# fircarpediem/LSS2_Multimodal_nu

Hardware: AMD Instinct MI355X
Metric: BEV frames/sec (6-cam 352x128 -> 200x200x64), full hot path: CamEncode lift + splat + BevEncode (higher is better)
Workload: dtype bf16; 1 GPU; BASELINE configs[1]: model_BEV_TXT LSS hot path, batch=4/GPU, 6 cams 352x128, D=41, 200x200x64 BEV -> BevEncode -> 200x200x4, trunk (EfficientNet) not included: features are the input; batch_per_gpu=4, global_batch=4, parallelism=dp1 (sample-sharded, no collective), precision=bf16

## Files before the change

lss2_multimodal_nu_amd/csrc/conv_ring.hip:

```cpp
#include <stdlib.h>

#include <type_traits>

#include "lss_common.h"

namespace {

constexpr int RK_SW = 20, RK_SH = 4;
constexpr int RK_PW = 24, RK_PH = 6;
constexpr int RK_KC = 32;
constexpr int RK_POSB = RK_KC * 2;
constexpr int RK_STRIP_PATCH = RK_PH * RK_PW * RK_POSB;
constexpr int RK_SLAB = 128 * RK_KC * 2;
constexpr int RK_SRC_H = 5, RK_SRC_W = 14;
constexpr int RK_SRC_STRIP = RK_SRC_H * RK_SRC_W * RK_POSB;

struct RingArgs {
  const unsigned short* x;
  const unsigned short* x2;
  const unsigned char* w;
  const float* scale;
  const float* shift;
  unsigned short* y;
  const float* head_w;
  const float* head_b;
  float* head_out;
  int head_n;
  int B, H, W, Cx, C2, up, Hin, Win, Cin, Cout, relu, wt;
  float ry, rx;
  int SX, SY, nstrips, nblk, nch;
  unsigned long long* stats;
};

__device__ __attribute__((aligned(128))) unsigned char lss_ring_zero_page[128];
__device__ int lss_ring_timeouts;

template <int MODE, bool HEAD, int NSL>
struct RingLds {
  static constexpr int RING = 0;
  static constexpr int PATCH = NSL * RK_SLAB;
  static constexpr int SRC = PATCH + 2 * 4 * RK_STRIP_PATCH;
  static constexpr int HEADX = SRC + (MODE == 1 ? 4 * RK_SRC_STRIP : 0);
  static constexpr int FLAGS = HEADX + (HEAD ? 4 * 80 * 4 * 4 : 0);
  static constexpr int TOTAL = FLAGS + 256;
};
constexpr int F_FULL_W = 0, F_FREE_W = 8, F_FULL_P = 16, F_FREE_P = 18, F_HEAD = 20, F_FULL_S = 24, F_FREE_S = 25;

#define RK_TIMEOUT_COUNTER lss_ring_timeouts
#include "ring_prims.h"

typedef __attribute__((ext_vector_type(2))) float rk_f32x2;
typedef __attribute__((ext_vector_type(2))) __bf16 rk_bf16x2;
__device__ __forceinline__ unsigned int rk_pack_bf2(float lo, float hi) {
  const rk_f32x2 v = {lo, hi};
  return __builtin_bit_cast(unsigned int, __builtin_convertvector(v, rk_bf16x2));
}
__device__ __forceinline__ uint4 rk_blend(const uint4& q00, const uint4& q01, const uint4& q10, const uint4& q11,
                                          float lx, float ly) {
  const float w11 = lx * ly, w10 = ly - w11, w01 = lx - w11, w00 = 1.f - lx - ly + w11;
  const unsigned int* u00 = reinterpret_cast<const unsigned int*>(&q00);
  const unsigned int* u01 = reinterpret_cast<const unsigned int*>(&q01);
  const unsigned int* u10 = reinterpret_cast<const unsigned int*>(&q10);
  const unsigned int* u11 = reinterpret_cast<const unsigned int*>(&q11);
  uint4 out;
  unsigned int* o = reinterpret_cast<unsigned int*>(&out);
#pragma unroll
  for (int i = 0; i < 4; ++i) {
    float lo = __builtin_bit_cast(float, u00[i] << 16) * w00;
    float hi = __builtin_bit_cast(float, u00[i] & 0xffff0000u) * w00;
    lo = __builtin_fmaf(__builtin_bit_cast(float, u01[i] << 16), w01, lo);
    hi = __builtin_fmaf(__builtin_bit_cast(float, u01[i] & 0xffff0000u), w01, hi);
    lo = __builtin_fmaf(__builtin_bit_cast(float, u10[i] << 16), w10, lo);
    hi = __builtin_fmaf(__builtin_bit_cast(float, u10[i] & 0xffff0000u), w10, hi);
    lo = __builtin_fmaf(__builtin_bit_cast(float, u11[i] << 16), w11, lo);
    hi = __builtin_fmaf(__builtin_bit_cast(float, u11[i] & 0xffff0000u), w11, hi);
    o[i] = rk_pack_bf2(lo, hi);
  }
  return out;
}

#ifndef RK_PSLEEP
#define RK_PSLEEP 8
#endif
#ifndef RK_PRIO_C
#define RK_PRIO_C 0
#endif
#ifndef RK_PRIO_P
#define RK_PRIO_P 3
#endif
#ifndef RK_PRIO_W
#define RK_PRIO_W 2
#endif
constexpr int RK_NS = 4;
constexpr int RK_NCONS = 2 * RK_NS;
constexpr int RK_NPATCH = 3;
constexpr int RK_NWAVES = RK_NCONS + 1 + RK_NPATCH;
constexpr int RK_NPIECE = RK_NS * 9;

struct RingTile {
  int nb;
  int b[RK_NS], oy0[RK_NS], ox0[RK_NS];
  bool ok[RK_NS];
};

template <int MODE, bool HEAD, int NSL>
__global__ __launch_bounds__(RK_NWAVES * 64, 3) void conv_ring_kernel(RingArgs a) {
  using L = RingLds<MODE, HEAD, NSL>;
  constexpr int LA = NSL - 2;
  static_assert(NSL >= 3 && NSL <= 8, "ring depth");
  static_assert(L::TOTAL <= 160 * 1024, "LDS of one CU");
  __shared__ __attribute__((aligned(1024))) unsigned char smem[L::TOTAL];
  const int tid = threadIdx.x, lane = tid & 63;
  const int wave = __builtin_amdgcn_readfirstlane(tid >> 6);
  const rk_flag_t flags = (rk_flag_t)((__attribute__((address_space(3))) unsigned char*)smem + L::FLAGS);
  if (tid < 64) flags[tid] = 0;
  __syncthreads();
  int st0 = 0, st1 = 0;
#ifdef RK_STATS
#define RK_ST(x) x
  const unsigned long long t_entry = a.stats ? __builtin_amdgcn_s_memrealtime() : 0ull;
  auto write_stats = [&]() {
    if (a.stats != nullptr && lane == 0) {
      unsigned long long* o = a.stats + ((size_t)blockIdx.x * RK_NWAVES + wave) * 6;
      o[0] = (unsigned long long)st0; o[1] = (unsigned long long)st1;
      o[2] = __builtin_amdgcn_s_memrealtime() - t_entry; o[3] = t_entry;
    }
  };
#else
#define RK_ST(x)
  auto write_stats = [&]() {};
#endif

  RingTile T;
  {
    const int nwg = gridDim.x, bid = blockIdx.x;
    const int xcd = bid & 7, q8 = nwg >> 3, r8 = nwg & 7;
    const int t = (xcd < r8 ? xcd * (q8 + 1) : r8 * (q8 + 1) + (xcd - r8) * q8) + (bid >> 3);
    T.nb = t % a.nblk;
    const int quad = t / a.nblk;
#pragma unroll
    for (int s = 0; s < RK_NS; ++s) {
      int sid = RK_NS * quad + s;
      T.ok[s] = sid < a.nstrips;
      sid = min(sid, a.nstrips - 1);
      const int per = a.SX * a.SY;
      T.b[s] = sid / per;
      const int rem = sid - T.b[s] * per;
      const int sy = rem / a.SX;
      T.oy0[s] = sy * RK_SH;
      T.ox0[s] = (rem - sy * a.SX) * RK_SW;
    }
  }
  const int nsteps = a.nch * 9;

  if (wave == RK_NCONS) {
    __builtin_amdgcn_s_setprio(RK_PRIO_W);
    const unsigned char* wsrc = a.w + (size_t)T.nb * a.nch * 9 * RK_SLAB + lane * 16;
    int slot = 0, gen = 1, pslot = 0, pgen = 1, inflight = 0;
    auto publish_oldest = [&]() {
      switch (inflight) {
        case 1: rk_wait_vmcnt<0>(); break;
        case 2: rk_wait_vmcnt<8>(); break;
        case 3: rk_wait_vmcnt<16>(); break;
        case 4: rk_wait_vmcnt<24>(); break;
        case 5: rk_wait_vmcnt<32>(); break;
        case 6: rk_wait_vmcnt<40>(); break;
        default: rk_wait_vmcnt<48>(); break;
      }
      rk_set(flags + F_FULL_W + pslot, pgen, lane);
      if (++pslot == NSL) { pslot = 0; ++pgen; }
      --inflight;
    };
    for (int i = 0; i < nsteps; ++i) {
      if (gen > 1) {
        int spins = 0;
        while (rk_peek(flags + F_FREE_W + slot) < RK_NCONS * (gen - 1)) {
          if (inflight > 0) {
            publish_oldest();
          } else {
            __builtin_amdgcn_s_sleep(1);
            ++st0;
            if (++spins > RK_SPIN_LIMIT) {
              if (lane == 0) atomicAdd(&lss_ring_timeouts, 1);
              break;
            }
          }
        }
        asm volatile("" ::: "memory");
      }
      unsigned char* dst = smem + L::RING + slot * RK_SLAB;
#ifndef RK_DIAG_NOWDMA
#pragma unroll
      for (int k = 0; k < 8; ++k) rk_glds16(wsrc + (size_t)i * RK_SLAB + k * 1024, dst + k * 1024);
#endif
      ++inflight;
      if (inflight > LA) publish_oldest();
      if (++slot == NSL) { slot = 0; ++gen; }
    }
    while (inflight > 0) publish_oldest();
    rk_wait_vmcnt<0>();
    write_stats();
    return;
  }

  if (wave > RK_NCONS) {
    __builtin_amdgcn_s_setprio(RK_PRIO_P);
    const int pw = wave - RK_NCONS - 1;
    constexpr int NIT = RK_NPIECE / RK_NPATCH;
    const int nskip = MODE == 1 ? a.C2 / RK_KC : a.nch;
    const unsigned short* xfull = MODE == 1 ? a.x2 : a.x;
    const int cfull = MODE == 1 ? a.C2 : a.Cx;
    int poff[NIT];
    int g_off[MODE == 1 ? NIT : 1];
    unsigned int g_w[MODE == 1 ? NIT : 1];
    constexpr int NSRC = MODE == 1 ? (RK_NS * 5 + RK_NPATCH - 1) / RK_NPATCH : 1;
    int src_o[NSRC];
#pragma unroll
    for (int k = 0; k < NIT; ++k) {
      const int it = pw + k * RK_NPATCH;
      const int s = it / 9, pos = (it % 9) * 16 + (lane >> 2);
      const int prow = pos / RK_PW, pcol = pos - prow * RK_PW;
      const int piece = (lane & 3) ^ ((prow & 1) << 1);
      const int sb = s == 0 ? T.b[0] : s == 1 ? T.b[1] : s == 2 ? T.b[2] : T.b[3];
      const int soy = s == 0 ? T.oy0[0] : s == 1 ? T.oy0[1] : s == 2 ? T.oy0[2] : T.oy0[3];
      const int sox = s == 0 ? T.ox0[0] : s == 1 ? T.ox0[1] : s == 2 ? T.ox0[2] : T.ox0[3];
      const bool sok = s == 0 ? T.ok[0] : s == 1 ? T.ok[1] : s == 2 ? T.ok[2] : T.ok[3];
      const int iy = soy - 1 + prow, ix = sox - 1 + pcol;
      const bool in = sok && pcol < RK_SW + 2 && iy >= 0 && iy < a.Hin && ix >= 0 && ix < a.Win;
      poff[k] = (in && cfull > 0) ? ((sb * a.Hin + iy) * a.Win + ix) * cfull + piece * 8 : -1;
      if (MODE == 1) {
        g_off[k] = 0;
        g_w[k] = 0;
        if (in) {
          const int wy0 = (int)(a.ry * (float)max(soy - 1, 0)), wx0 = (int)(a.rx * (float)max(sox - 1, 0));
          const float sy = a.ry * (float)iy, sx = a.rx * (float)ix;
          const int y0 = (int)sy, x0 = (int)sx;
          const unsigned int wy = (unsigned int)((sy - (float)y0) * 65536.f + 0.5f);
          const unsigned int wx = (unsigned int)((sx - (float)x0) * 65536.f + 0.5f);
          g_w[k] = min(wx, 65535u) | (min(wy, 65535u) << 16);
          const int fl = (x0 < a.W - 1 ? 1 : 0) | (y0 < a.H - 1 ? 2 : 0) | 4;
          g_off[k] = ((((y0 - wy0) * RK_SRC_W + (x0 - wx0)) * 4 + piece) * 16) | fl;
        }
      }
    }
    if (MODE == 1) {
#pragma unroll
      for (int k = 0; k < NSRC; ++k) {
        const int it = pw + k * RK_NPATCH;
        const int s = min(it / 5, RK_NS - 1), q = (it % 5) * 64 + lane;
        const int pos = min(q >> 2, RK_SRC_H * RK_SRC_W - 1), part = q & 3;
        const int sr = pos / RK_SRC_W, sc = pos - sr * RK_SRC_W;
        const int sb = s == 0 ? T.b[0] : s == 1 ? T.b[1] : s == 2 ? T.b[2] : T.b[3];
        const int soy = s == 0 ? T.oy0[0] : s == 1 ? T.oy0[1] : s == 2 ? T.oy0[2] : T.oy0[3];
        const int sox = s == 0 ? T.ox0[0] : s == 1 ? T.ox0[1] : s == 2 ? T.ox0[2] : T.ox0[3];
        const int wy0 = (int)(a.ry * (float)max(soy - 1, 0)), wx0 = (int)(a.rx * (float)max(sox - 1, 0));
        src_o[k] = ((sb * a.H + min(wy0 + sr, a.H - 1)) * a.W + min(wx0 + sc, a.W - 1)) * a.Cx + part * 8;
      }
    }
    auto issue_full = [&](int c, int buf) {
      unsigned char* dst = smem + L::PATCH + buf * (RK_NS * RK_STRIP_PATCH);
#pragma unroll
      for (int k = 0; k < NIT; ++k) {
        const void* src = poff[k] >= 0 ? (const void*)(xfull + poff[k] + c * RK_KC) : (const void*)lss_ring_zero_page;
        rk_glds16(src, dst + (pw + k * RK_NPATCH) * 1024);
      }
    };
    if (MODE == 0) {
      issue_full(0, 0);
      if (a.nch > 1) {
        issue_full(1, 1);
        rk_wait_vmcnt<NIT>();
      } else {
        rk_wait_vmcnt<0>();
      }
      rk_add1(flags + F_FULL_P + 0, lane);
      for (int c = 0; c < a.nch; ++c) {
        if (c + 1 < a.nch) {
          rk_wait_vmcnt<0>();
          rk_add1(flags + F_FULL_P + ((c + 1) & 1), lane);
        }
        if (c + 2 < a.nch) {
          st0 += rk_wait_ge<RK_PSLEEP>(flags + F_FREE_P + (c & 1), RK_NCONS * ((c >> 1) + 1));
          issue_full(c + 2, c & 1);
        }
      }
    } else {
      auto issue_src = [&](int c) {
        const int cx = c * RK_KC - a.C2;
#pragma unroll
        for (int k = 0; k < NSRC; ++k) {
          const int it = pw + k * RK_NPATCH;
          if (it < RK_NS * 5 && (it % 5) * 64 + lane < RK_SRC_H * RK_SRC_W * 4)
            rk_glds16(a.x + src_o[k] + cx, smem + L::SRC + (it / 5) * RK_SRC_STRIP + (it % 5) * 1024);
        }
      };
      auto prepare = [&](int c) {
        if (c < nskip) {
          st0 += rk_wait_ge<RK_PSLEEP>(flags + F_FREE_P + (c & 1), RK_NCONS * (c >> 1));
          issue_full(c, c & 1);
        } else {
          st1 += rk_wait_ge(flags + F_FREE_S, RK_NPATCH * (c - nskip));
          issue_src(c);
        }
      };
      prepare(0);
      for (int c = 0; c < a.nch; ++c) {
        rk_wait_vmcnt<0>();
        if (c >= nskip) {
          rk_add1(flags + F_FULL_S, lane);
          st1 += rk_wait_ge(flags + F_FULL_S, RK_NPATCH * (c - nskip + 1));
          st0 += rk_wait_ge<RK_PSLEEP>(flags + F_FREE_P + (c & 1), RK_NCONS * (c >> 1));
          unsigned char* dst = smem + L::PATCH + (c & 1) * (RK_NS * RK_STRIP_PATCH);
          uint4 qa[4], qb[4];
          auto corners = [&](int k, uint4* q) {
            const int it = pw + k * RK_NPATCH;
            const unsigned char* p00 = smem + L::SRC + (it / 9) * RK_SRC_STRIP + (g_off[k] & 0xfff0);
            const int dx = (g_off[k] & 1) ? 4 * 16 : 0, dy = (g_off[k] & 2) ? RK_SRC_W * 4 * 16 : 0;
            q[0] = *reinterpret_cast<const uint4*>(p00);
#if defined(RK_DIAG_ONEREAD)
            q[1] = q[0]; q[2] = q[0]; q[3] = q[0];
            asm volatile("" : "+v"(q[1].x), "+v"(q[2].x), "+v"(q[3].x));
#else
            q[1] = *reinterpret_cast<const uint4*>(p00 + dx);
            q[2] = *reinterpret_cast<const uint4*>(p00 + dy);
            q[3] = *reinterpret_cast<const uint4*>(p00 + dy + dx);
#endif
          };
          auto finish = [&](int k, const uint4* q) {
            uint4 v = make_uint4(0, 0, 0, 0);
#ifndef RK_DIAG_NOBLEND
#if defined(RK_DIAG_READSONLY)
            v.x = q[0].x ^ q[1].x ^ q[2].x ^ q[3].x; v.y = q[0].y ^ q[1].y ^ q[2].y ^ q[3].y;
            v.z = q[0].z ^ q[1].z ^ q[2].z ^ q[3].z; v.w = q[0].w ^ q[1].w ^ q[2].w ^ q[3].w;
#else
            v = rk_blend(q[0], q[1], q[2], q[3], (float)(g_w[k] & 0xffff) * (1.f / 65536.f),
                         (float)(g_w[k] >> 16) * (1.f / 65536.f));
#endif
            const bool in = (g_off[k] & 4) != 0;
            v.x = in ? v.x : 0u; v.y = in ? v.y : 0u; v.z = in ? v.z : 0u; v.w = in ? v.w : 0u;
#endif
            *reinterpret_cast<uint4*>(dst + (pw + k * RK_NPATCH) * 1024 + lane * 16) = v;
          };
          corners(0, qa);
#pragma unroll
          for (int k = 0; k < NIT; k += 2) {
            corners(k + 1, qb);
            finish(k, qa);
            if (k + 2 < NIT) corners(k + 2, qa);
            finish(k + 1, qb);
          }
          rk_wait_lgkm0();
          rk_add1(flags + F_FREE_S, lane);
        }
        if (c + 1 < a.nch && c + 1 >= nskip) prepare(c + 1);
        rk_add1(flags + F_FULL_P + (c & 1), lane);
        if (c + 1 < a.nch && c + 1 < nskip) prepare(c + 1);
      }
    }
    rk_wait_vmcnt<0>();
    write_stats();
    return;
  }

  __builtin_amdgcn_s_setprio(RK_PRIO_C);
  const int sidx = wave >> 1, cg = wave & 1;
  const int n = lane & 15, kq = lane >> 4;
  const int my_b = sidx == 0 ? T.b[0] : sidx == 1 ? T.b[1] : sidx == 2 ? T.b[2] : T.b[3];
  const int my_oy0 = sidx == 0 ? T.oy0[0] : sidx == 1 ? T.oy0[1] : sidx == 2 ? T.oy0[2] : T.oy0[3];
  const int my_ox0 = sidx == 0 ? T.ox0[0] : sidx == 1 ? T.ox0[1] : sidx == 2 ? T.ox0[2] : T.ox0[3];
  const bool my_ok = sidx == 0 ? T.ok[0] : sidx == 1 ? T.ok[1] : sidx == 2 ? T.ok[2] : T.ok[3];
  f32x4 acc[5][4];
#pragma unroll
  for (int j = 0; j < 5; ++j)
#pragma unroll
    for (int t = 0; t < 4; ++t) acc[j][t] = (f32x4){0.f, 0.f, 0.f, 0.f};
  bf16x8 fw[4], fp[5];
#define RK_DSR(dst, addr, off) asm volatile("ds_read_b128 %0, %1 offset:%2" : "=v"(dst) : "v"(addr), "n"(off))
  const unsigned int lanepk =
      (unsigned int)(cg * 4096 + lane * 16) |
      ((unsigned int)((((n >> 2) * RK_PW + (n & 3)) * RK_POSB + (kq << 4)) ^ (((n >> 2) & 1) << 5)) << 16);
  const unsigned int flag_base = (unsigned int)(__UINTPTR_TYPE__)flags;
  const int pconst = L::PATCH + sidx * RK_STRIP_PATCH;
  auto add1 = [&](int word) {
    unsigned long long save;
    asm volatile("s_mov_b64 %0, exec\n\ts_mov_b64 exec, 1\n\tds_add_u32 %1, %2\n\ts_mov_b64 exec, %0"
                 : "=&s"(save)
                 : "v"(flag_base + 4 * word), "v"(1)
                 : "memory");
  };

  RK_ST(const unsigned long long tc_loop = __builtin_amdgcn_s_memtime(); const unsigned long long tr_loop = __builtin_amdgcn_s_memrealtime();)
  int slot = 0, gen = 1, buf = 0, pgen = 1;
  rk_wait_ge(flags + F_FULL_P + 0, RK_NPATCH);
  rk_wait_ge(flags + F_FULL_W + 0, 1);
  int fnext;
  {
    const int wa = (int)(lanepk & 0xffffu) + L::RING, pa = (int)(lanepk >> 16) + pconst;
    RK_DSR(fw[0], wa, 0);
    RK_DSR(fw[1], wa, 1024);
    asm volatile("ds_read_b32 %0, %1" : "=v"(fnext) : "v"(flag_base + 4 * (F_FULL_W + (1 % NSL))));
    RK_DSR(fp[0], pa, 0 * 4 * RK_POSB);
    RK_DSR(fp[1], pa, 1 * 4 * RK_POSB);
    RK_DSR(fp[2], pa, 2 * 4 * RK_POSB);
    RK_DSR(fp[3], pa, 3 * 4 * RK_POSB);
    RK_DSR(fp[4], pa, 4 * 4 * RK_POSB);
  }

  auto step = [&](auto TAPc, bool last) {
    constexpr int TAP = decltype(TAPc)::value;
    constexpr int NT = (TAP + 1) % 9;
    constexpr int POFF = (NT / 3) * (RK_PW * RK_POSB) + (NT % 3) * RK_POSB;
    {
      const int wa = (int)(lanepk & 0xffffu) + (L::RING + slot * RK_SLAB);
      RK_DSR(fw[2], wa, 2048);
      RK_DSR(fw[3], wa, 3072);
    }
    __builtin_amdgcn_sched_barrier(0);
    asm volatile("s_waitcnt lgkmcnt(6)" : "+v"(fw[0]), "+v"(fw[1]), "+v"(fp[0]));
    acc[0][0] = __builtin_amdgcn_mfma_f32_16x16x32_bf16(fw[0], fp[0], acc[0][0], 0, 0, 0);
    acc[0][1] = __builtin_amdgcn_mfma_f32_16x16x32_bf16(fw[1], fp[0], acc[0][1], 0, 0, 0);
    __builtin_amdgcn_sched_barrier(0);
    int nslot = slot + 1, ngen = gen;
    if (nslot == NSL) { nslot = 0; ++ngen; }
    int nbuf = buf, npgen = pgen;
    if (TAP == 8) {
      nbuf = buf ^ 1;
      if (nbuf == 0) ++npgen;
    }
    const int wan = (int)(lanepk & 0xffffu) + (L::RING + nslot * RK_SLAB);
    __builtin_amdgcn_sched_barrier(0);
    asm volatile("s_waitcnt lgkmcnt(5)" : "+v"(fp[1]));
    acc[1][0] = __builtin_amdgcn_mfma_f32_16x16x32_bf16(fw[0], fp[1], acc[1][0], 0, 0, 0);
    acc[1][1] = __builtin_amdgcn_mfma_f32_16x16x32_bf16(fw[1], fp[1], acc[1][1], 0, 0, 0);
    __builtin_amdgcn_sched_barrier(0);
    const int pan = (int)((lanepk >> 16) ^ (NT / 3 == 1 ? 32u : 0u)) + (pconst + nbuf * (RK_NS * RK_STRIP_PATCH));
    const int n2 = nslot + 1 == NSL ? 0 : nslot + 1;
    const unsigned int fa = flag_base + 4 * (F_FULL_W + n2);
    __builtin_amdgcn_sched_barrier(0);
    asm volatile("s_waitcnt lgkmcnt(4)" : "+v"(fp[2]));
    acc[2][0] = __builtin_amdgcn_mfma_f32_16x16x32_bf16(fw[0], fp[2], acc[2][0], 0, 0, 0);
    acc[2][1] = __builtin_amdgcn_mfma_f32_16x16x32_bf16(fw[1], fp[2], acc[2][1], 0, 0, 0);
    __builtin_amdgcn_sched_barrier(0);
    asm volatile("s_waitcnt lgkmcnt(3)" : "+v"(fp[3]));
    acc[3][0] = __builtin_amdgcn_mfma_f32_16x16x32_bf16(fw[0], fp[3], acc[3][0], 0, 0, 0);
    acc[3][1] = __builtin_amdgcn_mfma_f32_16x16x32_bf16(fw[1], fp[3], acc[3][1], 0, 0, 0);
    __builtin_amdgcn_sched_barrier(0);
    asm volatile("s_waitcnt lgkmcnt(2)" : "+v"(fp[4]));
    acc[4][0] = __builtin_amdgcn_mfma_f32_16x16x32_bf16(fw[0], fp[4], acc[4][0], 0, 0, 0);
    acc[4][1] = __builtin_amdgcn_mfma_f32_16x16x32_bf16(fw[1], fp[4], acc[4][1], 0, 0, 0);
    __builtin_amdgcn_sched_barrier(0);
    if (!last) {
      if (__builtin_amdgcn_readfirstlane(fnext) < ngen) st0 += 1 + rk_wait_ge(flags + F_FULL_W + nslot, ngen);
      if (TAP == 8) st1 += rk_wait_ge(flags + F_FULL_P + nbuf, RK_NPATCH * npgen);
      asm volatile("" ::: "memory");
      RK_DSR(fw[0], wan, 0);
      RK_DSR(fw[1], wan, 1024);
      asm volatile("ds_read_b32 %0, %1" : "=v"(fnext) : "v"(fa));
      __builtin_amdgcn_sched_barrier(0);
      asm volatile("s_waitcnt lgkmcnt(3)" : "+v"(fw[2]), "+v"(fw[3]));
    } else {
      asm volatile("s_waitcnt lgkmcnt(0)" : "+v"(fw[2]), "+v"(fw[3]));
    }
    acc[0][2] = __builtin_amdgcn_mfma_f32_16x16x32_bf16(fw[2], fp[0], acc[0][2], 0, 0, 0);
    acc[0][3] = __builtin_amdgcn_mfma_f32_16x16x32_bf16(fw[3], fp[0], acc[0][3], 0, 0, 0);
    __builtin_amdgcn_sched_barrier(0);
    add1(F_FREE_W + slot);
    if (!last) RK_DSR(fp[0], pan, POFF + 0 * 4 * RK_POSB);
    __builtin_amdgcn_sched_barrier(0);
    acc[1][2] = __builtin_amdgcn_mfma_f32_16x16x32_bf16(fw[2], fp[1], acc[1][2], 0, 0, 0);
    acc[1][3] = __builtin_amdgcn_mfma_f32_16x16x32_bf16(fw[3], fp[1], acc[1][3], 0, 0, 0);
    __builtin_amdgcn_sched_barrier(0);
    if (!last) RK_DSR(fp[1], pan, POFF + 1 * 4 * RK_POSB);
    __builtin_amdgcn_sched_barrier(0);
    acc[2][2] = __builtin_amdgcn_mfma_f32_16x16x32_bf16(fw[2], fp[2], acc[2][2], 0, 0, 0);
    acc[2][3] = __builtin_amdgcn_mfma_f32_16x16x32_bf16(fw[3], fp[2], acc[2][3], 0, 0, 0);
    __builtin_amdgcn_sched_barrier(0);
    if (!last) RK_DSR(fp[2], pan, POFF + 2 * 4 * RK_POSB);
    __builtin_amdgcn_sched_barrier(0);
    acc[3][2] = __builtin_amdgcn_mfma_f32_16x16x32_bf16(fw[2], fp[3], acc[3][2], 0, 0, 0);
    acc[3][3] = __builtin_amdgcn_mfma_f32_16x16x32_bf16(fw[3], fp[3], acc[3][3], 0, 0, 0);
    __builtin_amdgcn_sched_barrier(0);
    if (!last) RK_DSR(fp[3], pan, POFF + 3 * 4 * RK_POSB);
    __builtin_amdgcn_sched_barrier(0);
    acc[4][2] = __builtin_amdgcn_mfma_f32_16x16x32_bf16(fw[2], fp[4], acc[4][2], 0, 0, 0);
    acc[4][3] = __builtin_amdgcn_mfma_f32_16x16x32_bf16(fw[3], fp[4], acc[4][3], 0, 0, 0);
    __builtin_amdgcn_sched_barrier(0);
    if (!last) RK_DSR(fp[4], pan, POFF + 4 * 4 * RK_POSB);
    if (TAP == 8) add1(F_FREE_P + buf);
    __builtin_amdgcn_sched_barrier(0);
    slot = nslot; gen = ngen; buf = nbuf; pgen = npgen;
  };
  for (int c = 0; c < a.nch; ++c) {
    step(std::integral_constant<int, 0>{}, false);
    step(std::integral_constant<int, 1>{}, false);
    step(std::integral_constant<int, 2>{}, false);
    step(std::integral_constant<int, 3>{}, false);
    step(std::integral_constant<int, 4>{}, false);
    step(std::integral_constant<int, 5>{}, false);
    step(std::integral_constant<int, 6>{}, false);
    step(std::integral_constant<int, 7>{}, false);
    step(std::integral_constant<int, 8>{}, c + 1 == a.nch);
  }
#undef RK_DSR
  RK_ST(if (a.stats != nullptr && lane == 0) { unsigned long long* o = a.stats + ((size_t)blockIdx.x * RK_NWAVES + wave) * 6; o[2] = __builtin_amdgcn_s_memrealtime() - t_entry; o[4] = __builtin_amdgcn_s_memtime() - tc_loop; o[5] = __builtin_amdgcn_s_memrealtime() - tr_loop; })

  const int ch0 = T.nb * 128 + cg * 64 + kq * 16;
  {
    float sc[16], sh[16];
#pragma unroll
    for (int v4 = 0; v4 < 4; ++v4) {
      f32x4 s4 = {1.f, 1.f, 1.f, 1.f}, h4 = {0.f, 0.f, 0.f, 0.f};
      if (a.scale) s4 = *reinterpret_cast<const f32x4*>(a.scale + ch0 + v4 * 4);
      if (a.shift) h4 = *reinterpret_cast<const f32x4*>(a.shift + ch0 + v4 * 4);
#pragma unroll
      for (int i = 0; i < 4; ++i) { sc[v4 * 4 + i] = s4[i]; sh[v4 * 4 + i] = h4[i]; }
    }
#pragma unroll
    for (int j = 0; j < 5; ++j)
#pragma unroll
      for (int t = 0; t < 4; ++t)
#pragma unroll
        for (int i = 0; i < 4; ++i) {
          float v = acc[j][t][i] * sc[t * 4 + i] + sh[t * 4 + i];
          acc[j][t][i] = a.relu ? fmaxf(v, 0.f) : v;
        }
  }
  const int oy = my_oy0 + (n >> 2);
  if (!HEAD) {
    typedef __attribute__((ext_vector_type(4))) unsigned int u32x4;
    const __amdgpu_buffer_rsrc_t yrsrc = __builtin_amdgcn_make_buffer_rsrc(
        a.y, 0, a.wt ? (int)((size_t)a.B * a.Hin * a.Win * a.Cout * 2) : 0, 0x00020000);
    typedef __attribute__((ext_vector_type(2))) unsigned int u32x2;
    const int chs = T.nb * 128 + cg * 64 + kq * 8;
#pragma unroll
    for (int j = 0; j < 5; ++j) {
      const int ox = my_ox0 + j * 4 + (n & 3);
      u32x4 ox_[2];
#pragma unroll
      for (int d = 0; d < 4; ++d) {
        const unsigned lo = rk_pack_bf2(acc[j][d >> 1][(d & 1) * 2], acc[j][d >> 1][(d & 1) * 2 + 1]);
        const unsigned hi = rk_pack_bf2(acc[j][2 + (d >> 1)][(d & 1) * 2], acc[j][2 + (d >> 1)][(d & 1) * 2 + 1]);
        const u32x2 r = __builtin_amdgcn_permlane16_swap(lo, hi, false, false);
        const u32x2 t = __builtin_amdgcn_permlane32_swap(r[0], r[1], false, false);
        ox_[0][d] = t[0];
        ox_[1][d] = t[1];
      }
      if (!my_ok || oy >= a.Hin || ox >= a.Win) continue;
      const size_t o = (((size_t)my_b * a.Hin + oy) * a.Win + ox) * a.Cout + chs;
#pragma unroll
      for (int hf = 0; hf < 2; ++hf) {
        if (a.wt) __builtin_amdgcn_raw_buffer_store_b128(ox_[hf], yrsrc, (int)((o + hf * 32) * 2), 0, 16);
        else *reinterpret_cast<u32x4*>(a.y + o + hf * 32) = ox_[hf];
      }
    }
  } else {
    float part[5];
#pragma unroll
    for (int j = 0; j < 5; ++j) part[j] = 0.f;
    const int c0 = cg * 64 + kq * 16;
#pragma unroll 1
    for (int k = 0; k < 4; ++k) {
      float hw[16];
#pragma unroll
      for (int v4 = 0; v4 < 4; ++v4) {
        f32x4 w4 = {0.f, 0.f, 0.f, 0.f};
        if (k < a.head_n) w4 = *reinterpret_cast<const f32x4*>(a.head_w + (size_t)k * 128 + c0 + v4 * 4);
#pragma unroll
        for (int i = 0; i < 4; ++i) hw[v4 * 4 + i] = w4[i];
      }
#pragma unroll
      for (int j = 0; j < 5; ++j) {
        float s = 0.f;
#pragma unroll
        for (int t = 0; t < 4; ++t)
#pragma unroll
          for (int i = 0; i < 4; ++i) s = fmaf(acc[j][t][i], hw[t * 4 + i], s);
        s += __shfl_xor(s, 16, 64);
        s += __shfl_xor(s, 32, 64);
        if (kq == k) part[j] = s;
      }
    }
    float* hx = reinterpret_cast<float*>(smem + L::HEADX) + sidx * (80 * 4);
    if (cg == 1) {
#pragma unroll
      for (int j = 0; j < 5; ++j) hx[(j * 16 + n) * 4 + kq] = part[j];
      rk_wait_lgkm0();
      rk_set(flags + F_HEAD + sidx, 1, lane);
    } else {
      rk_wait_ge(flags + F_HEAD + sidx, 1);
      if (kq < a.head_n) {
        const float hb = a.head_b[kq];
#pragma unroll
        for (int j = 0; j < 5; ++j) {
          const int ox = my_ox0 + j * 4 + (n & 3);
          const float v = part[j] + hx[(j * 16 + n) * 4 + kq] + hb;
          if (my_ok && oy < a.Hin && ox < a.Win)
            a.head_out[(((size_t)my_b * a.head_n + kq) * a.Hin + oy) * a.Win + ox] = v;
        }
      }
    }
  }
  RK_ST(if (a.stats != nullptr && lane == 0) {
    unsigned long long* o = a.stats + ((size_t)blockIdx.x * RK_NWAVES + wave) * 6;
    o[0] = (unsigned long long)st0; o[1] = (unsigned long long)st1; o[3] = t_entry;
  })
#undef RK_ST
}

template <bool DGRAD>
__global__ void pack_weights_ring_kernel(const float* __restrict__ w, int Cout, int Cin, unsigned short* __restrict__ out) {
  const size_t n = (size_t)Cout * Cin * 9;
  const int nch = Cin / RK_KC;
  for (size_t e = (size_t)blockIdx.x * 256 + threadIdx.x; e < n; e += (size_t)gridDim.x * 256) {
    const int j = e & 7;
    size_t r = e >> 3;
    const int l = r & 63; r >>= 6;
    const int t = r & 3; r >>= 2;
    const int cg = r & 1; r >>= 1;
    const int tap = r % 9; r /= 9;
    const int chunk = r % nch;
    const int nb = r / nch;
    const int co = nb * 128 + cg * 64 + ((l & 15) >> 2) * 16 + 4 * t + (l & 3);
    const int ci = chunk * RK_KC + (l >> 4) * 8 + j;
    out[e] = lss_f2bf(DGRAD ? w[((size_t)ci * Cout + co) * 9 + (8 - tap)] : w[((size_t)co * Cin + ci) * 9 + tap]);
  }
}

}

extern "C" int lss_conv2d_ring_ok(int B, int H, int W, int Cx, int C2, int up, int Cout, int head_n) {
  if (B <= 0 || H <= 0 || W <= 0 || Cx <= 0 || C2 < 0 || up <= 0 || Cout <= 0 || head_n < 0) return 0;
  if (Cout % 128 != 0 || Cx % 32 != 0 || C2 % 32 != 0) return 0;
  if (head_n > 0 && (Cout != 128 || head_n > 4)) return 0;
  const bool fused = up > 1 || C2 > 0;
  const int Hin = H * up, Win = W * up;
  if (fused) {
    if (up < 2) return 0;
    const float ry = Hin > 1 ? (float)(H - 1) / (float)(Hin - 1) : 0.f, rx = Win > 1 ? (float)(W - 1) / (float)(Win - 1) : 0.f;
    if ((int)(ry * (RK_PH - 1) + 0.999f) + 2 > RK_SRC_H || (int)(rx * (RK_SW + 1) + 0.999f) + 2 > RK_SRC_W) return 0;
  }
  if ((long long)B * Hin * Win * (long long)Cout >= (1LL << 31) / 2) return 0;
  if ((long long)B * H * W * (long long)Cx >= (1LL << 31) || (long long)B * Hin * Win * (long long)(C2 > 0 ? C2 : 1) >= (1LL << 31))
    return 0;
  const long long strips = (long long)B * lss_cdiv(Hin, RK_SH) * lss_cdiv(Win, RK_SW);
  return strips / RK_NS * (Cout / 128) >= 96 ? 1 : 0;
}

extern "C" int lss_conv2d_ring_timeouts(void) {
  int v = -1;
  if (hipMemcpyFromSymbol(&v, HIP_SYMBOL(lss_ring_timeouts), sizeof(int), 0, hipMemcpyDeviceToHost) != hipSuccess) return -1;
  return v;
}

extern "C" size_t lss_conv2d_ring_packed_weight_bytes(int Cout, int Cin) {
  if (Cout <= 0 || Cin <= 0 || Cout % 128 != 0 || Cin % RK_KC != 0) return 0;
  return (size_t)Cout * Cin * 9 * 2;
}

extern "C" int lss_conv2d_pack_weights_ring(const float* w_oihw, int Cout, int Cin, void* w_packed, void* stream) {
  LSS_CHECK_PTR(w_oihw); LSS_CHECK_PTR(w_packed);
  if (lss_conv2d_ring_packed_weight_bytes(Cout, Cin) == 0) return LSS_E_SHAPE;
  const size_t n = (size_t)Cout * Cin * 9;
  const int grid = (int)((n + 255) / 256 > 4096 ? 4096 : (n + 255) / 256);
  hipLaunchKernelGGL(pack_weights_ring_kernel<false>, dim3(grid), dim3(256), 0, lss_stream(stream), w_oihw, Cout, Cin,
                     reinterpret_cast<unsigned short*>(w_packed));
  return lss_launch_status();
}

extern "C" int lss_conv2d_pack_weights_ring_dgrad(const float* w_oihw, int Cout, int Cin, void* w_packed, void* stream) {
  LSS_CHECK_PTR(w_oihw); LSS_CHECK_PTR(w_packed);
  if (lss_conv2d_ring_packed_weight_bytes(Cin, Cout) == 0) return LSS_E_SHAPE;
  const size_t n = (size_t)Cout * Cin * 9;
  const int grid = (int)((n + 255) / 256 > 4096 ? 4096 : (n + 255) / 256);
  hipLaunchKernelGGL(pack_weights_ring_kernel<true>, dim3(grid), dim3(256), 0, lss_stream(stream), w_oihw, Cin, Cout,
                     reinterpret_cast<unsigned short*>(w_packed));
  return lss_launch_status();
}

int lss_conv_ring_launch(const void* x, const void* x2, const void* w_ring, const float* scale, const float* shift,
                         void* y, const float* head_w, const float* head_b, float* head_out, int head_n, int B, int H,
                         int W, int Cx, int C2, int up, int Cout, int relu, int wt, hipStream_t st) {
  if (!lss_conv2d_ring_ok(B, H, W, Cx, C2, up, Cout, head_n)) return LSS_E_SHAPE;
  if (relu != 0 && relu != 1) return LSS_E_LAYOUT;
  RingArgs a;
  a.x = reinterpret_cast<const unsigned short*>(x);
  a.x2 = reinterpret_cast<const unsigned short*>(x2);
  a.w = reinterpret_cast<const unsigned char*>(w_ring);
  a.scale = scale; a.shift = shift;
  a.y = reinterpret_cast<unsigned short*>(y);
  a.head_w = head_w; a.head_b = head_b; a.head_out = head_out; a.head_n = head_n;
  a.B = B; a.H = H; a.W = W; a.Cx = Cx; a.C2 = C2; a.up = up;
  a.Hin = H * up; a.Win = W * up; a.Cin = Cx + C2; a.Cout = Cout; a.relu = relu; a.wt = wt;
  a.ry = a.Hin > 1 ? (float)(H - 1) / (float)(a.Hin - 1) : 0.f;
  a.rx = a.Win > 1 ? (float)(W - 1) / (float)(a.Win - 1) : 0.f;
  a.SX = lss_cdiv(a.Win, RK_SW); a.SY = lss_cdiv(a.Hin, RK_SH);
  a.nstrips = B * a.SX * a.SY;
  a.nblk = Cout / 128;
  a.nch = a.Cin / RK_KC;
  {
    const char* e = getenv("LSS_RING_STATS");
    a.stats = e ? reinterpret_cast<unsigned long long*>(strtoull(e, nullptr, 16)) : nullptr;
  }
  const bool fused = up > 1 || C2 > 0;
  const dim3 g((a.nstrips + RK_NS - 1) / RK_NS * a.nblk), blk(RK_NWAVES * 64);
  if (head_n > 0) {
    if (fused) hipLaunchKernelGGL((conv_ring_kernel<1, true, 7>), g, blk, 0, st, a);
    else hipLaunchKernelGGL((conv_ring_kernel<0, true, 8>), g, blk, 0, st, a);
  } else {
    if (fused) hipLaunchKernelGGL((conv_ring_kernel<1, false, 7>), g, blk, 0, st, a);
    else hipLaunchKernelGGL((conv_ring_kernel<0, false, 8>), g, blk, 0, st, a);
  }
  return lss_launch_status();
}
```

Before: 10750 frames/s.

## Share one 2x2-strip input tile per block in fused upsample conv

```diff
diff --git a/lss2_multimodal_nu_amd/csrc/conv_ring.hip b/lss2_multimodal_nu_amd/csrc/conv_ring.hip
--- a/lss2_multimodal_nu_amd/csrc/conv_ring.hip
+++ b/lss2_multimodal_nu_amd/csrc/conv_ring.hip
@@ -14,6 +14,12 @@
 constexpr int RK_SLAB = 128 * RK_KC * 2;
 constexpr int RK_SRC_H = 5, RK_SRC_W = 14;
 constexpr int RK_SRC_STRIP = RK_SRC_H * RK_SRC_W * RK_POSB;
+constexpr int RK_TH = 2 * RK_SH, RK_TW = 2 * RK_SW;
+constexpr int RK_TPW = RK_TW + 2, RK_TPH = RK_TH + 2;
+constexpr int RK_TPIECE = (RK_TPH * RK_TPW * 4 + 63) / 64;
+constexpr int RK_TSRC_H = 7, RK_TSRC_W = 23;
+constexpr int RK_TSRC = RK_TSRC_H * RK_TSRC_W * RK_POSB;
+constexpr int RK_TSRC_PIECE = (RK_TSRC_H * RK_TSRC_W * 4 + 63) / 64;
 
 struct RingArgs {
   const unsigned short* x;
@@ -35,12 +41,13 @@
 __device__ __attribute__((aligned(128))) unsigned char lss_ring_zero_page[128];
 __device__ int lss_ring_timeouts;
 
-template <int MODE, bool HEAD, int NSL>
+template <int MODE, bool HEAD, int NSL, bool T22>
 struct RingLds {
   static constexpr int RING = 0;
   static constexpr int PATCH = NSL * RK_SLAB;
-  static constexpr int SRC = PATCH + 2 * 4 * RK_STRIP_PATCH;
-  static constexpr int HEADX = SRC + (MODE == 1 ? 4 * RK_SRC_STRIP : 0);
+  static constexpr int PBUF = T22 ? RK_TPIECE * 1024 : 4 * RK_STRIP_PATCH;
+  static constexpr int SRC = PATCH + 2 * PBUF;
+  static constexpr int HEADX = SRC + (MODE == 1 ? (T22 ? RK_TSRC : 4 * RK_SRC_STRIP) : 0);
   static constexpr int FLAGS = HEADX + (HEAD ? 4 * 80 * 4 * 4 : 0);
   static constexpr int TOTAL = FLAGS + 256;
 };
@@ -95,7 +102,6 @@
 constexpr int RK_NCONS = 2 * RK_NS;
 constexpr int RK_NPATCH = 3;
 constexpr int RK_NWAVES = RK_NCONS + 1 + RK_NPATCH;
-constexpr int RK_NPIECE = RK_NS * 9;
 
 struct RingTile {
   int nb;
@@ -103,9 +109,11 @@
   bool ok[RK_NS];
 };
 
-template <int MODE, bool HEAD, int NSL>
+template <int MODE, bool HEAD, int NSL, bool T22>
 __global__ __launch_bounds__(RK_NWAVES * 64, 3) void conv_ring_kernel(RingArgs a) {
-  using L = RingLds<MODE, HEAD, NSL>;
+  static_assert(!T22 || MODE == 1, "shared tile: fused upsample only");
+  using L = RingLds<MODE, HEAD, NSL, T22>;
+  constexpr int PW = T22 ? RK_TPW : RK_PW;
   constexpr int LA = NSL - 2;
   static_assert(NSL >= 3 && NSL <= 8, "ring depth");
   static_assert(L::TOTAL <= 160 * 1024, "LDS of one CU");
@@ -138,17 +146,29 @@
     const int t = (xcd < r8 ? xcd * (q8 + 1) : r8 * (q8 + 1) + (xcd - r8) * q8) + (bid >> 3);
     T.nb = t % a.nblk;
     const int quad = t / a.nblk;
-#pragma unroll
-    for (int s = 0; s < RK_NS; ++s) {
-      int sid = RK_NS * quad + s;
-      T.ok[s] = sid < a.nstrips;
-      sid = min(sid, a.nstrips - 1);
-      const int per = a.SX * a.SY;
-      T.b[s] = sid / per;
-      const int rem = sid - T.b[s] * per;
-      const int sy = rem / a.SX;
-      T.oy0[s] = sy * RK_SH;
-      T.ox0[s] = (rem - sy * a.SX) * RK_SW;
+    if (T22) {
+      const int tx = a.SX >> 1, per = tx * (a.SY >> 1);
+      const int b = quad / per, rem = quad - b * per, ty = rem / tx;
+#pragma unroll
+      for (int s = 0; s < RK_NS; ++s) {
+        T.ok[s] = true;
+        T.b[s] = b;
+        T.oy0[s] = ty * RK_TH + (s >> 1) * RK_SH;
+        T.ox0[s] = (rem - ty * tx) * RK_TW + (s & 1) * RK_SW;
+      }
+    } else {
+#pragma unroll
+      for (int s = 0; s < RK_NS; ++s) {
+        int sid = RK_NS * quad + s;
+        T.ok[s] = sid < a.nstrips;
+        sid = min(sid, a.nstrips - 1);
+        const int per = a.SX * a.SY;
+        T.b[s] = sid / per;
+        const int rem = sid - T.b[s] * per;
+        const int sy = rem / a.SX;
+        T.oy0[s] = sy * RK_SH;
+        T.ox0[s] = (rem - sy * a.SX) * RK_SW;
+      }
     }
   }
   const int nsteps = a.nch * 9;
@@ -206,40 +226,52 @@
   if (wave > RK_NCONS) {
     __builtin_amdgcn_s_setprio(RK_PRIO_P);
     const int pw = wave - RK_NCONS - 1;
-    constexpr int NIT = RK_NPIECE / RK_NPATCH;
+    constexpr int NIT = (T22 ? RK_TPIECE : RK_NS * 9) / RK_NPATCH;
+    static_assert(NIT * RK_NPATCH == (T22 ? RK_TPIECE : RK_NS * 9), "pieces split evenly over the patch loaders");
     const int nskip = MODE == 1 ? a.C2 / RK_KC : a.nch;
     const unsigned short* xfull = MODE == 1 ? a.x2 : a.x;
     const int cfull = MODE == 1 ? a.C2 : a.Cx;
     int poff[NIT];
     int g_off[MODE == 1 ? NIT : 1];
-    unsigned int g_w[MODE == 1 ? NIT : 1];
-    constexpr int NSRC = MODE == 1 ? (RK_NS * 5 + RK_NPATCH - 1) / RK_NPATCH : 1;
+    constexpr int NWD = MODE == 1 && T22 ? NIT : 1, NWP = MODE == 1 && !T22 ? NIT : 1;
+    float g_lx[NWD], g_ly[NWD];
+    unsigned int g_wp[NWP];
+    constexpr int SRCW = T22 ? RK_TSRC_W : RK_SRC_W;
+    constexpr int NSRCP = T22 ? RK_TSRC_PIECE : RK_NS * 5;
+    constexpr int NSRC = MODE == 1 ? (NSRCP + RK_NPATCH - 1) / RK_NPATCH : 1;
     int src_o[NSRC];
 #pragma unroll
     for (int k = 0; k < NIT; ++k) {
       const int it = pw + k * RK_NPATCH;
-      const int s = it / 9, pos = (it % 9) * 16 + (lane >> 2);
-      const int prow = pos / RK_PW, pcol = pos - prow * RK_PW;
+      const int s = T22 ? 0 : it / 9, pos = T22 ? it * 16 + (lane >> 2) : (it % 9) * 16 + (lane >> 2);
+      const int prow = pos / PW, pcol = pos - prow * PW;
       const int piece = (lane & 3) ^ ((prow & 1) << 1);
       const int sb = s == 0 ? T.b[0] : s == 1 ? T.b[1] : s == 2 ? T.b[2] : T.b[3];
       const int soy = s == 0 ? T.oy0[0] : s == 1 ? T.oy0[1] : s == 2 ? T.oy0[2] : T.oy0[3];
       const int sox = s == 0 ? T.ox0[0] : s == 1 ? T.ox0[1] : s == 2 ? T.ox0[2] : T.ox0[3];
       const bool sok = s == 0 ? T.ok[0] : s == 1 ? T.ok[1] : s == 2 ? T.ok[2] : T.ok[3];
       const int iy = soy - 1 + prow, ix = sox - 1 + pcol;
-      const bool in = sok && pcol < RK_SW + 2 && iy >= 0 && iy < a.Hin && ix >= 0 && ix < a.Win;
+      const bool used = T22 ? pos < RK_TPH * RK_TPW : pcol < RK_SW + 2;
+      const bool in = sok && used && iy >= 0 && iy < a.Hin && ix >= 0 && ix < a.Win;
       poff[k] = (in && cfull > 0) ? ((sb * a.Hin + iy) * a.Win + ix) * cfull + piece * 8 : -1;
       if (MODE == 1) {
         g_off[k] = 0;
-        g_w[k] = 0;
+        unsigned int g_w = 0;
         if (in) {
           const int wy0 = (int)(a.ry * (float)max(soy - 1, 0)), wx0 = (int)(a.rx * (float)max(sox - 1, 0));
           const float sy = a.ry * (float)iy, sx = a.rx * (float)ix;
           const int y0 = (int)sy, x0 = (int)sx;
           const unsigned int wy = (unsigned int)((sy - (float)y0) * 65536.f + 0.5f);
           const unsigned int wx = (unsigned int)((sx - (float)x0) * 65536.f + 0.5f);
-          g_w[k] = min(wx, 65535u) | (min(wy, 65535u) << 16);
+          g_w = min(wx, 65535u) | (min(wy, 65535u) << 16);
           const int fl = (x0 < a.W - 1 ? 1 : 0) | (y0 < a.H - 1 ? 2 : 0) | 4;
-          g_off[k] = ((((y0 - wy0) * RK_SRC_W + (x0 - wx0)) * 4 + piece) * 16) | fl;
+          g_off[k] = ((((y0 - wy0) * SRCW + (x0 - wx0)) * 4 + piece) * 16) | fl;
+        }
+        if constexpr (T22) {
+          g_lx[k] = (float)(g_w & 0xffff) * (1.f / 65536.f);
+          g_ly[k] = (float)(g_w >> 16) * (1.f / 65536.f);
+        } else {
+          g_wp[k] = g_w;
         }
       }
     }
@@ -247,9 +279,9 @@
 #pragma unroll
       for (int k = 0; k < NSRC; ++k) {
         const int it = pw + k * RK_NPATCH;
-        const int s = min(it / 5, RK_NS - 1), q = (it % 5) * 64 + lane;
-        const int pos = min(q >> 2, RK_SRC_H * RK_SRC_W - 1), part = q & 3;
-        const int sr = pos / RK_SRC_W, sc = pos - sr * RK_SRC_W;
+        const int s = T22 ? 0 : min(it / 5, RK_NS - 1), q = (T22 ? it : it % 5) * 64 + lane;
+        const int pos = min(q >> 2, (T22 ? RK_TSRC_H : RK_SRC_H) * SRCW - 1), part = q & 3;
+        const int sr = pos / SRCW, sc = pos - sr * SRCW;
         const int sb = s == 0 ? T.b[0] : s == 1 ? T.b[1] : s == 2 ? T.b[2] : T.b[3];
         const int soy = s == 0 ? T.oy0[0] : s == 1 ? T.oy0[1] : s == 2 ? T.oy0[2] : T.oy0[3];
         const int sox = s == 0 ? T.ox0[0] : s == 1 ? T.ox0[1] : s == 2 ? T.ox0[2] : T.ox0[3];
@@ -258,7 +290,7 @@
       }
     }
     auto issue_full = [&](int c, int buf) {
-      unsigned char* dst = smem + L::PATCH + buf * (RK_NS * RK_STRIP_PATCH);
+      unsigned char* dst = smem + L::PATCH + buf * L::PBUF;
 #pragma unroll
       for (int k = 0; k < NIT; ++k) {
         const void* src = poff[k] >= 0 ? (const void*)(xfull + poff[k] + c * RK_KC) : (const void*)lss_ring_zero_page;
@@ -290,8 +322,12 @@
 #pragma unroll
         for (int k = 0; k < NSRC; ++k) {
           const int it = pw + k * RK_NPATCH;
-          if (it < RK_NS * 5 && (it % 5) * 64 + lane < RK_SRC_H * RK_SRC_W * 4)
+          if (T22) {
+            if (it < RK_TSRC_PIECE && it * 64 + lane < RK_TSRC_H * RK_TSRC_W * 4)
+              rk_glds16(a.x + src_o[k] + cx, smem + L::SRC + it * 1024);
+          } else if (it < RK_NS * 5 && (it % 5) * 64 + lane < RK_SRC_H * RK_SRC_W * 4) {
             rk_glds16(a.x + src_o[k] + cx, smem + L::SRC + (it / 5) * RK_SRC_STRIP + (it % 5) * 1024);
+          }
         }
       };
       auto prepare = [&](int c) {
@@ -310,12 +346,12 @@
           rk_add1(flags + F_FULL_S, lane);
           st1 += rk_wait_ge(flags + F_FULL_S, RK_NPATCH * (c - nskip + 1));
           st0 += rk_wait_ge<RK_PSLEEP>(flags + F_FREE_P + (c & 1), RK_NCONS * (c >> 1));
-          unsigned char* dst = smem + L::PATCH + (c & 1) * (RK_NS * RK_STRIP_PATCH);
+          unsigned char* dst = smem + L::PATCH + (c & 1) * L::PBUF;
           uint4 qa[4], qb[4];
           auto corners = [&](int k, uint4* q) {
             const int it = pw + k * RK_NPATCH;
-            const unsigned char* p00 = smem + L::SRC + (it / 9) * RK_SRC_STRIP + (g_off[k] & 0xfff0);
-            const int dx = (g_off[k] & 1) ? 4 * 16 : 0, dy = (g_off[k] & 2) ? RK_SRC_W * 4 * 16 : 0;
+            const unsigned char* p00 = smem + L::SRC + (T22 ? 0 : (it / 9) * RK_SRC_STRIP) + (g_off[k] & 0xfff0);
+            const int dx = (g_off[k] & 1) ? 4 * 16 : 0, dy = (g_off[k] & 2) ? SRCW * 4 * 16 : 0;
             q[0] = *reinterpret_cast<const uint4*>(p00);
 #if defined(RK_DIAG_ONEREAD)
             q[1] = q[0]; q[2] = q[0]; q[3] = q[0];
@@ -333,8 +369,11 @@
             v.x = q[0].x ^ q[1].x ^ q[2].x ^ q[3].x; v.y = q[0].y ^ q[1].y ^ q[2].y ^ q[3].y;
             v.z = q[0].z ^ q[1].z ^ q[2].z ^ q[3].z; v.w = q[0].w ^ q[1].w ^ q[2].w ^ q[3].w;
 #else
-            v = rk_blend(q[0], q[1], q[2], q[3], (float)(g_w[k] & 0xffff) * (1.f / 65536.f),
-                         (float)(g_w[k] >> 16) * (1.f / 65536.f));
+            if constexpr (T22)
+              v = rk_blend(q[0], q[1], q[2], q[3], g_lx[k], g_ly[k]);
+            else
+              v = rk_blend(q[0], q[1], q[2], q[3], (float)(g_wp[k] & 0xffff) * (1.f / 65536.f),
+                           (float)(g_wp[k] >> 16) * (1.f / 65536.f));
 #endif
             const bool in = (g_off[k] & 4) != 0;
             v.x = in ? v.x : 0u; v.y = in ? v.y : 0u; v.z = in ? v.z : 0u; v.w = in ? v.w : 0u;
@@ -344,10 +383,12 @@
           corners(0, qa);
 #pragma unroll
           for (int k = 0; k < NIT; k += 2) {
-            corners(k + 1, qb);
+            if (k + 1 < NIT) corners(k + 1, qb);
             finish(k, qa);
-            if (k + 2 < NIT) corners(k + 2, qa);
-            finish(k + 1, qb);
+            if (k + 1 < NIT) {
+              if (k + 2 < NIT) corners(k + 2, qa);
+              finish(k + 1, qb);
+            }
           }
           rk_wait_lgkm0();
           rk_add1(flags + F_FREE_S, lane);
@@ -378,9 +419,9 @@
 #define RK_DSR(dst, addr, off) asm volatile("ds_read_b128 %0, %1 offset:%2" : "=v"(dst) : "v"(addr), "n"(off))
   const unsigned int lanepk =
       (unsigned int)(cg * 4096 + lane * 16) |
-      ((unsigned int)((((n >> 2) * RK_PW + (n & 3)) * RK_POSB + (kq << 4)) ^ (((n >> 2) & 1) << 5)) << 16);
+      ((unsigned int)((((n >> 2) * PW + (n & 3)) * RK_POSB + (kq << 4)) ^ (((n >> 2) & 1) << 5)) << 16);
   const unsigned int flag_base = (unsigned int)(__UINTPTR_TYPE__)flags;
-  const int pconst = L::PATCH + sidx * RK_STRIP_PATCH;
+  const int pconst = L::PATCH + (T22 ? ((sidx >> 1) * RK_SH * PW + (sidx & 1) * RK_SW) * RK_POSB : sidx * RK_STRIP_PATCH);
   auto add1 = [&](int word) {
     unsigned long long save;
     asm volatile("s_mov_b64 %0, exec\n\ts_mov_b64 exec, 1\n\tds_add_u32 %1, %2\n\ts_mov_b64 exec, %0"
@@ -409,7 +450,7 @@
   auto step = [&](auto TAPc, bool last) {
     constexpr int TAP = decltype(TAPc)::value;
     constexpr int NT = (TAP + 1) % 9;
-    constexpr int POFF = (NT / 3) * (RK_PW * RK_POSB) + (NT % 3) * RK_POSB;
+    constexpr int POFF = (NT / 3) * (PW * RK_POSB) + (NT % 3) * RK_POSB;
     {
       const int wa = (int)(lanepk & 0xffffu) + (L::RING + slot * RK_SLAB);
       RK_DSR(fw[2], wa, 2048);
@@ -433,7 +474,7 @@
     acc[1][0] = __builtin_amdgcn_mfma_f32_16x16x32_bf16(fw[0], fp[1], acc[1][0], 0, 0, 0);
     acc[1][1] = __builtin_amdgcn_mfma_f32_16x16x32_bf16(fw[1], fp[1], acc[1][1], 0, 0, 0);
     __builtin_amdgcn_sched_barrier(0);
-    const int pan = (int)((lanepk >> 16) ^ (NT / 3 == 1 ? 32u : 0u)) + (pconst + nbuf * (RK_NS * RK_STRIP_PATCH));
+    const int pan = (int)((lanepk >> 16) ^ (NT / 3 == 1 ? 32u : 0u)) + (pconst + nbuf * L::PBUF);
     const int n2 = nslot + 1 == NSL ? 0 : nslot + 1;
     const unsigned int fa = flag_base + 4 * (F_FULL_W + n2);
     __builtin_amdgcn_sched_barrier(0);
@@ -702,13 +743,17 @@
     a.stats = e ? reinterpret_cast<unsigned long long*>(strtoull(e, nullptr, 16)) : nullptr;
   }
   const bool fused = up > 1 || C2 > 0;
+  const bool t22 = fused && a.Hin % RK_TH == 0 && a.Win % RK_TW == 0 &&
+                   (int)(a.ry * (RK_TPH - 1) + 0.999f) + 2 <= RK_TSRC_H && (int)(a.rx * (RK_TPW - 1) + 0.999f) + 2 <= RK_TSRC_W;
   const dim3 g((a.nstrips + RK_NS - 1) / RK_NS * a.nblk), blk(RK_NWAVES * 64);
   if (head_n > 0) {
-    if (fused) hipLaunchKernelGGL((conv_ring_kernel<1, true, 7>), g, blk, 0, st, a);
-    else hipLaunchKernelGGL((conv_ring_kernel<0, true, 8>), g, blk, 0, st, a);
+    if (t22) hipLaunchKernelGGL((conv_ring_kernel<1, true, 7, true>), g, blk, 0, st, a);
+    else if (fused) hipLaunchKernelGGL((conv_ring_kernel<1, true, 7, false>), g, blk, 0, st, a);
+    else hipLaunchKernelGGL((conv_ring_kernel<0, true, 8, false>), g, blk, 0, st, a);
   } else {
-    if (fused) hipLaunchKernelGGL((conv_ring_kernel<1, false, 7>), g, blk, 0, st, a);
-    else hipLaunchKernelGGL((conv_ring_kernel<0, false, 8>), g, blk, 0, st, a);
+    if (t22) hipLaunchKernelGGL((conv_ring_kernel<1, false, 7, true>), g, blk, 0, st, a);
+    else if (fused) hipLaunchKernelGGL((conv_ring_kernel<1, false, 7, false>), g, blk, 0, st, a);
+    else hipLaunchKernelGGL((conv_ring_kernel<0, false, 8, false>), g, blk, 0, st, a);
   }
   return lss_launch_status();
 }
```

Result: faster. 10970 frames/s (median of 6 runs) (+2.1%).
